# nzfeng/signed-heat-3d

Hardware: AMD Instinct MI355X
Metric: grid-nodes/sec end-to-end SHM (conv+PCG) (higher is better)
Workload: dtype f64 (Step 1: f64 / packed-f32 tiers)

## Files before the change

signed-heat-3d_amd/csrc/shm_conv_tiered.hip.h:

```cpp
#pragma once
#include "shm_far_carry.h"
#include "shm_kernels.hip.h"

namespace shm {

typedef unsigned uint2v __attribute__((ext_vector_type(2)));
constexpr double kNearA1 = 3.384507729693224e-04;
__device__ __forceinline__ double yukawa_near(double x, double c1, double c2, double m1, const uint2v* __restrict__ tab) {
    const double y0 = __builtin_amdgcn_rsq(x);
    const double t = x * y0;
    const double e2 = fma(-t, y0, 1.0);
    const double cc = fma(e2, c2, c1);
    const double tm = fma(-t, cc, m1);
    const double kf = tm - m1;
    const unsigned ki = (unsigned)__double_as_longlong(tm);
    const double f = fma(-t, cc, -kf);
    const double q = y0 * cc;
    double p = 5.727446245172041e-08;
    p = fma(p, f, kNearA1);
    p = fma(p, f, 1.0);
    uint2v tv = tab[ki & 2047u];
    tv.y += ki << 9;
    return __builtin_bit_cast(double, tv) * (p * q);
}

template <int B>
__device__ __forceinline__ void yukawa_near_batch(const double* __restrict__ x, double c1, double c2, double m1, const uint2v* __restrict__ tab, double* __restrict__ g) {
    double y0[B], t[B], cc[B], q[B], tm[B], f[B], p[B];
    unsigned ki[B];
    uint2v tv[B];
#pragma unroll
    for (int b = 0; b < B; b++) y0[b] = __builtin_amdgcn_rsq(x[b]);
#pragma unroll
    for (int b = 0; b < B; b++) t[b] = x[b] * y0[b];
#pragma unroll
// ... 111 lines not shown
#define SHM_TIER_WAVES_PER_EU 2
#endif
template <int NPT, typename TY, bool CHECK>
__global__ __launch_bounds__(kBlock) __attribute__((amdgpu_waves_per_eu(SHM_TIER_WAVES_PER_EU, SHM_TIER_WAVES_PER_EU))) void conv_tiered_kernel(
    ConvParams P, const double* __restrict__ src , const float* __restrict__ clusters,
    const double* __restrict__ exp_tab_g , TY* __restrict__ Y0, TY* __restrict__ Y1, TY* __restrict__ Y2,
    unsigned long long* __restrict__ counters, unsigned* __restrict__ next_unit ) {
    static_assert(NPT % 2 == 0, "the far tier handles a lane's nodes in packed pairs");
    constexpr int kWaves = kBlock / kWave;
    constexpr int kFarUnroll = SHM_TIER_FAR_UNROLL;
    static_assert(kFarUnroll == kFarGroup, "the carry's bookkeeping (shm_far_carry.h) counts in groups of the far loop's unroll");
    constexpr int kFarList = kTierCluster + kFarGroup;
    static_assert((kTierCluster + kFarGroup - 1 + kFarGroup - 1) / kFarGroup * kFarGroup <= kFarList, "carry + cluster + padding fit the far lists");
    __shared__ double stage64[kWaves][kTierCluster * 6];
    __shared__ __attribute__((aligned(16))) float farA[kWaves][kFarList * 4];
    __shared__ __attribute__((aligned(16))) float farB[kWaves][kFarList * NPT];
    __shared__ __attribute__((aligned(16))) float farC[kWaves][kFarList * 2];
#if SHM_TIER_LDS_FETCH
    __shared__ double2 raw[kWaves][3][kTierCluster];
#endif
    __shared__ uint2v exp_tab[2048];
    __shared__ float4 star_stash[kWaves];
    const int wave = __builtin_amdgcn_readfirstlane((int)(threadIdx.x >> 6)), lane = (int)(threadIdx.x & 63);
    double* const tile = stage64[wave];
    float* const tA = farA[wave];
    float* const tB = farB[wave];
    float* const tC = farC[wave];
    for (int a = threadIdx.x; a < 2048; a += kBlock) {
        uint2v tv = __builtin_bit_cast(uint2v, exp_tab_g[a]);
        tv.y -= (unsigned)a << 9;
        exp_tab[a] = tv;
    }
    __syncthreads();
    const int n = P.n;
    const size_t plane = (size_t)n * n;
    const float lam_l2 = (float)(P.lambda * 1.4426950408889634);
    const float g_l2 = P.tier_log * 1.4426950408889634f;
    const bool drop_on = P.drop_eps_soft > 0.f;
    const float cellq = (float)(P.cell * (P.lambda * 1.4426950408889634));
    const float lws = uniform_f32((float)log2(P.wscale));
    constexpr double kHalfZ = 0.5 * (NPT - 1);
    constexpr double kHalfX = 0.5 * (kTierTX - 1), kHalfY = 0.5 * (kTierTY - 1);
    const float rt_w = (float)(sqrt(kHalfX * kHalfX + kHalfY * kHalfY + kHalfZ * kHalfZ) * P.cell) * 1.000001f;
    const float hx = uniform_f32((float)(kHalfX * P.cell) * 1.000001f), hy = uniform_f32((float)(kHalfY * P.cell) * 1.000001f),
                hz = uniform_f32((float)(kHalfZ * P.cell) * 1.000001f);
    const double c1 = -P.cexp, c2 = -0.5 * P.cexp;
    unsigned long long cnt_near = 0, cnt_far = 0, cnt_redo = 0;
    int decided = -1;
    const unsigned n_units = (unsigned)P.n_tiles;
    const unsigned per_q = (n_units + 7u) / 8u;
    const unsigned my_q = blockIdx.x & 7u;
    unsigned q_off = 0;
    for (;;) {
        unsigned unit = 0xffffffffu;
        while (q_off < 8u) {
            const unsigned q = (my_q + q_off) & 7u;
            const unsigned lo = q * per_q, hi = min(n_units, lo + per_q);
            unsigned t = 0;
            if (lane == 0) t = atomicAdd(next_unit + q, 1u);
            t = (unsigned)__builtin_amdgcn_readfirstlane((int)t);
            if (lo + t < hi) {
                unit = lo + t;
                break;
            }
            q_off++;
        }
        if (unit == 0xffffffffu) break;
        const int tzq = (int)(unit / (unsigned)(P.tiles_x * P.tiles_y)), trem = (int)unit - tzq * (P.tiles_x * P.tiles_y);
        const int tz = P.layer_order ? P.layer_order[tzq] : tzq;
        bool use_diff = false;
// ... 79 lines not shown

        const int k0 = __builtin_amdgcn_readfirstlane((int)floor((double)d0_w * P.cexp * (1.0 / 2048.0)));
        const double m1 = 6755399441055744.0 - 2048.0 * (double)k0;
        auto far_scale = [&]() {
            float d = d0_w;
            asm volatile("" : "+v"(d));
            return exp2_tab(fma((double)d, P.cexp, -2048.0 * (double)k0), exp_tab) * (P.lambda * 1.4426950408889634) / P.wscale;
        };
        float2v fl[NPT / 2];
#pragma unroll
        for (int e = 0; e < NPT / 2; e++) fl[e] = float2v{0.f, 0.f};
        const float range_c = uniform_f32(2.f * rt_w * lam_l2 - 113.f - coff);
        float star_ux = 0.f, star_uy = 0.f, star_uz = 0.f, star_dc = 0.f, star_inv_d = 0.f;
        if constexpr (CHECK) {
            use_diff = use_diff && coff + 2.f * rt_w * lam_l2 <= 72.f;
        }
        if (use_diff || drop_on) {
            const float inv = dmin > 0.f ? 1.f / dmin : 0.f;
            star_ux = uniform_f32(nx * inv);
            star_uy = uniform_f32(ny * inv);
            star_uz = uniform_f32(nz * inv);
            star_dc = uniform_f32(dmin * 1.000001f);
            const float bx = fmaxf(fabsf(nx) - hx, 0.f), by = fmaxf(fabsf(ny) - hy, 0.f), bz = fmaxf(fabsf(nz) - hz, 0.f);
            const float db = sqrtf(bx * bx + by * by + bz * bz);
            star_inv_d = uniform_f32(dmin > 0.f && db > 0.f ? 1.f / db : __builtin_huge_valf());
        }
        float R_soft = 0.f, R_hard = 0.f;
        if constexpr (CHECK) {
            if (drop_on && lane == 0) star_stash[wave] = float4{(cx - nx) * lam_l2, (cy - ny) * lam_l2, (cz - nz) * lam_l2, wnear};
        }
        const float span_c = uniform_f32(2.f * rt_w * lam_l2 - coff - 960.f);
        int far_pending = 0;
        int carry = 0;
#pragma unroll 1
        for (int pass = 0; pass < 2; pass++) {
#if SHM_TIER_LDS_FETCH
        auto fetch_cluster = [&](int c) {
            const char* g = reinterpret_cast<const char*>(src) + (size_t)c * (kTierCluster * 48);
            const unsigned lo = (unsigned)lane * 48u;
            __builtin_amdgcn_global_load_lds(g + lo, &raw[wave][0][0], 16, 0, 0);
            __builtin_amdgcn_global_load_lds(g + 16 + lo, &raw[wave][1][0], 16, 0, 0);
            __builtin_amdgcn_global_load_lds(g + 32 + lo, &raw[wave][2][0], 16, 0, 0);
        };
#else
        double nq[6];
        auto fetch_cluster = [&](int c) {
            const double* qn = src + ((size_t)c * kTierCluster + lane) * 6;
#pragma unroll
            for (int a = 0; a < 6; a++) nq[a] = qn[a];
        };
#endif
        int cur_batch = -1;
        unsigned long long kept_mask = 0ull, cdrop_mask = 0ull;
        auto load_batch = [&](int b) {
            cur_batch = b;
            const int ci = b * kWave + lane;
            const bool in = ci < P.n_clusters;
            const unsigned long long validm = __ballot(in);
            cdrop_mask = 0ull;
            if (drop_on) {
                const float2* rec = reinterpret_cast<const float2*>(clusters + (size_t)min(ci, P.n_clusters - 1) * kConvClusterRec);
                const float2 r0 = rec[0], r1 = rec[1], r2 = rec[2];
                const float gdx = cx - r0.x, gdy = cy - r0.y, gdz = cz - r1.x;
                const float gap = sqrtf(gdx * gdx + gdy * gdy + gdz * gdz) * 0.999999f - rt_w - r1.y - r_hi_w;
                const float lrel = lws - lnear_w - gap * lam_l2;
                const float lbmax = fmaf(r2.x, 1.4426950408889634f, lrel) + 2e-5f;
                const bool cand = in && gap > 0.f && lbmax <= P.drop_ltau;
                const unsigned long long candm = __ballot(cand);
                if (candm != 0ull) {
                    float bc = cand ? __builtin_amdgcn_exp2f(fmaf(r2.y, 1.4426950408889634f, lrel)) * (r_hi_w * __builtin_amdgcn_rcpf(r_hi_w + gap)) * 1.0001f : 0.f;
                    bc += __int_as_float(__builtin_amdgcn_ds_swizzle(__float_as_int(bc), 0x1f | (1 << 10)));
                    bc += __int_as_float(__builtin_amdgcn_ds_swizzle(__float_as_int(bc), 0x1f | (2 << 10)));
                    bc += __int_as_float(__builtin_amdgcn_ds_swizzle(__float_as_int(bc), 0x1f | (4 << 10)));
                    bc += __int_as_float(__builtin_amdgcn_ds_swizzle(__float_as_int(bc), 0x1f | (8 << 10)));
                    bc += __int_as_float(__builtin_amdgcn_ds_swizzle(__float_as_int(bc), 0x1f | (16 << 10)));
                    const float sum = __int_as_float(__builtin_amdgcn_readlane(__float_as_int(bc), 0)) + __int_as_float(__builtin_amdgcn_readlane(__float_as_int(bc), 32));
                    const float r_new = uniform_f32(R_soft + sum);
                    if (__builtin_amdgcn_readfirstlane((int)(r_new <= P.drop_eps_soft))) {
                        R_soft = r_new;
                        cdrop_mask = candm;
                    } else {
                        cdrop_mask = __ballot(cand && lbmax <= P.drop_ltau_hard);
                        R_hard = uniform_f32(R_hard + (float)(__builtin_popcountll(cdrop_mask) * kTierCluster) * P.drop_tau_hard);
                    }
                }
            }
            kept_mask = pass == 1 ? validm : validm & ~cdrop_mask;
        };
        auto next_kept = [&](int from, bool& cdrop) {
            cdrop = false;
#pragma unroll 1
            while (from < P.n_clusters) {
                const int b = from >> 6;
                if (b != cur_batch) load_batch(b);
                const unsigned long long m = kept_mask & (~0ull << (from & 63));
                if (m != 0ull) {
                    const int bit = (int)__builtin_ctzll(m);
                    cdrop = ((cdrop_mask >> bit) & 1ull) != 0ull;
                    return (b << 6) + bit;
                }
                from = (b + 1) << 6;
            }
            return P.n_clusters;
        };
        R_soft = 0.f;
        R_hard = 0.f;
        bool cdrop_cur = false, cdrop_next = false;
        int c = next_kept(0, cdrop_cur);
        if (c < P.n_clusters) fetch_cluster(c);
#pragma unroll 1
        while (c < P.n_clusters) {
            const int c_next = next_kept(c + 1, cdrop_next);
            const int c_fetch = c_next;
            double q[6];
#if SHM_TIER_LDS_FETCH
            {
                __builtin_amdgcn_s_waitcnt(0x0f70);
                const double2 r0 = raw[wave][0][lane], r1 = raw[wave][1][lane], r2 = raw[wave][2][lane];
                q[0] = r0.x; q[1] = r0.y; q[2] = r1.x; q[3] = r1.y; q[4] = r2.x; q[5] = r2.y;
                __builtin_amdgcn_s_waitcnt(0xc07f);
// ... 4 lines not shown
#endif
            if (c_fetch < P.n_clusters) fetch_cluster(c_fetch);
            unsigned long long nearmask, farmask;
            {
                float q32[6];
#pragma unroll
                for (int a = 0; a < 6; a++) q32[a] = a < 3 ? (float)q[a] : (float)(q[a] * P.wscale);
                const float dx = fmaxf(fabsf(cx - q32[0]) - hx, 0.f), dy = fmaxf(fabsf(cy - q32[1]) - hy, 0.f), dz = fmaxf(fabsf(cz - q32[2]) - hz, 0.f);
                const float dist = sqrtf(dx * dx + dy * dy + dz * dz);
                const float w2 = q32[3] * q32[3] + q32[4] * q32[4] + q32[5] * q32[5];
                const float lw = 0.5f * __log2f(w2);
                const float rel = lw + 1e-5f - lnear_w;
                const float lhs = (dist * 0.999999f - r_hi_w) * lam_l2;
                const bool valid = q[3] != 0. || q[4] != 0. || q[5] != 0.;
                const bool in_range = fmaf(dist, lam_l2, range_c) <= lw;
                float lhs_far = lhs, lhs_drop = lhs;
                {
                    bool want_diff = use_diff;
                    if (!want_diff && drop_on && !cdrop_cur) {
                        const float lb_box = rel - lhs;
                        want_diff = __ballot(valid && lb_box > P.drop_ltau && lb_box <= P.drop_ltau + 2.02f * rt_w * lam_l2) != 0ull;
                    }
                    if (want_diff) {
                        const float ex = cx - q32[0], ey = cy - q32[1], ez = cz - q32[2];
                        const float dc2 = ex * ex + ey * ey + ez * ez, rdc = __builtin_amdgcn_rsqf(dc2), dc = dc2 * rdc;
                        const float dot = (ex * star_ux + ey * star_uy + ez * star_uz) * rdc;
                        const float du = sqrtf(fmaxf(0.f, 2.f - 2.f * dot));
                        const float lip = du + rt_w * (__builtin_amdgcn_rcpf(dist) + star_inv_d);
                        const float lhs2 = (dc * 0.999999f - star_dc - rt_w * lip * 1.00001f) * lam_l2;
                        lhs_drop = fmaxf(lhs, lhs2);
                        if (use_diff) lhs_far = lhs_drop;
                    }
                }
                const bool far = lhs_far > g_l2 + rel && in_range && (!CHECK || dist >= r_hi_w);
                bool drop = valid && cdrop_cur;
                if (drop_on && !cdrop_cur) {
                    const float lb = rel - lhs_drop + 2e-5f;
                    const bool cand = valid && lb <= P.drop_ltau;
                    if (__ballot(cand) != 0ull) {
                        float bs = cand ? __builtin_amdgcn_exp2f(lb) * (r_hi_w * __builtin_amdgcn_rcpf(dist)) * 1.0001f : 0.f;
                        bs += __int_as_float(__builtin_amdgcn_ds_swizzle(__float_as_int(bs), 0x1f | (1 << 10)));
                        bs += __int_as_float(__builtin_amdgcn_ds_swizzle(__float_as_int(bs), 0x1f | (2 << 10)));
                        bs += __int_as_float(__builtin_amdgcn_ds_swizzle(__float_as_int(bs), 0x1f | (4 << 10)));
                        bs += __int_as_float(__builtin_amdgcn_ds_swizzle(__float_as_int(bs), 0x1f | (8 << 10)));
                        bs += __int_as_float(__builtin_amdgcn_ds_swizzle(__float_as_int(bs), 0x1f | (16 << 10)));
                        const float sum = __int_as_float(__builtin_amdgcn_readlane(__float_as_int(bs), 0)) + __int_as_float(__builtin_amdgcn_readlane(__float_as_int(bs), 32));
                        const float r_new = uniform_f32(R_soft + sum);
                        if (__builtin_amdgcn_readfirstlane((int)(r_new <= P.drop_eps_soft))) {
                            R_soft = r_new;
                            drop = cand;
                        } else {
                            drop = cand && lb <= P.drop_ltau_hard && dist >= r_hi_w;
                            R_hard = uniform_f32(R_hard + (float)__builtin_popcountll(__ballot(drop)) * P.drop_tau_hard);
                        }
                    }
                }
                const bool span_ok = fmaf(dist, lam_l2, span_c) < 0.f;
                const bool to64 = valid && (pass == 0 ? (!drop && !far) : (drop ? span_ok : true));
                const bool to32 = valid && pass == 0 && far && !drop;
                nearmask = __ballot(to64);
                farmask = __ballot(to32);
                if (to64) {
                    const int rnk = mask_rank(nearmask);
#pragma unroll
                    for (int a = 0; a < 6; a++) tile[rnk * 6 + a] = a < 3 ? q[a] : q[a] * P.cexp_inv;
                } else if (to32) {
                    const int rnk = carry + mask_rank(farmask);
                    *reinterpret_cast<float4*>(&tA[rnk * 4]) = float4{q32[0] * lam_l2, q32[1] * lam_l2, q32[3], q32[4]};
                    const float dz0 = qz0 - q32[2] * lam_l2;
                    float dz2[NPT];
#pragma unroll
                    for (int e = 0; e < NPT; e++) {
                        const float dz = e * cellq + dz0;
                        dz2[e] = dz * dz;
                    }
                    if constexpr (NPT == 4) *reinterpret_cast<float4*>(&tB[rnk * 4]) = float4{dz2[0], dz2[1], dz2[2], dz2[3]};
                    else *reinterpret_cast<float2*>(&tB[rnk * 2]) = float2{dz2[0], dz2[1]};
                    *reinterpret_cast<float2*>(&tC[rnk * 2]) = float2{q32[5], fabsf(q32[3]) + fabsf(q32[4]) + fabsf(q32[5])};
                }
            }
            const int nnear = __builtin_popcountll(nearmask), nfar = __builtin_popcountll(farmask);
            const FarCarryStep fs = far_carry_step(carry, nfar, far_pending, CHECK ? P.tier_flush : 0, c_next >= P.n_clusters);
            if (lane < fs.pad) {
                const int at = carry + nfar + lane;
                *reinterpret_cast<float4*>(&tA[at * 4]) = float4{1.0e18f, 1.0e18f, 0.f, 0.f};
#pragma unroll
                for (int e = 0; e < NPT; e++) tB[at * NPT + e] = 1.0e36f;
                *reinterpret_cast<float2*>(&tC[at * 2]) = float2{0.f, 0.f};
            }
            cnt_near += (unsigned)nnear;
            cnt_far += (unsigned)nfar;
            if (pass) cnt_redo += (unsigned)nnear;
            auto near_source = [&](const double (&rec)[6]) {
                const double dx = px - rec[0], dy = py - rec[1];
                const double dxy2 = dx * dx + dy * dy;
                const double dz0 = pz0 - rec[2];
                double x[NPT], g[NPT];
#pragma unroll
                for (int e = 0; e < NPT; e++) {
                    const double dz = e == 2 ? fma(2.0, P.cell, dz0) : e ? dz0 + e * P.cell : dz0;
                    x[e] = fma(dz, dz, dxy2);
                }
                constexpr int kB = SHM_TIER_NEAR_BATCH < NPT ? SHM_TIER_NEAR_BATCH : NPT;
#pragma unroll
                for (int b0 = 0; b0 < NPT; b0 += kB) yukawa_near_batch<kB>(x + b0, c1, c2, m1, exp_tab, g + b0);
#pragma unroll
                for (int e = 0; e < NPT; e++) {
                    ax[e] = fma(rec[3], g[e], ax[e]);
                    ay[e] = fma(rec[4], g[e], ay[e]);
                    az[e] = fma(rec[5], g[e], az[e]);
                }
            };
            for (int i0 = 0; i0 < nnear; i0++) {
                double rec[6];
#pragma unroll
                for (int a = 0; a < 6; a++) rec[a] = tile[6 * i0 + a];
                near_source(rec);
            }
            for (int i0f = 0; i0f < fs.run; i0f += kFarUnroll) {
                constexpr int kP = kFarUnroll * (NPT / 2);
                float2v wxy[kFarUnroll], pcw[kFarUnroll], d2[kP], rinv[kP], g[kP];
                float dxy2[kFarUnroll];
#pragma unroll
                for (int u = 0; u < kFarUnroll; u++) {
                    const int s = i0f + u;
// ... 34 lines not shown
                if (fs.flush) {
                    const double e0f = far_scale();
#pragma unroll
                    for (int e = 0; e < NPT; e++) {
                        ax[e] = fma((double)fx[e / 2][e & 1], e0f, ax[e]);
                        ay[e] = fma((double)fy[e / 2][e & 1], e0f, ay[e]);
                        az[e] = fma((double)fz[e / 2][e & 1], e0f, az[e]);
                    }
#pragma unroll
                    for (int e = 0; e < NPT / 2; e++) fx[e] = fy[e] = fz[e] = float2v{0.f, 0.f};
                }
            }
            if (fs.carry > 0 && fs.run > 0) {
                if (lane < fs.carry) {
                    const int from = fs.run + lane;
                    const float4 ca = *reinterpret_cast<const float4*>(&tA[from * 4]);
                    const float2 cc2 = *reinterpret_cast<const float2*>(&tC[from * 2]);
                    if constexpr (NPT == 4) {
                        const float4 cb = *reinterpret_cast<const float4*>(&tB[from * 4]);
                        *reinterpret_cast<float4*>(&tB[lane * 4]) = cb;
                    } else {
                        const float2 cb = *reinterpret_cast<const float2*>(&tB[from * 2]);
                        *reinterpret_cast<float2*>(&tB[lane * 2]) = cb;
                    }
                    *reinterpret_cast<float4*>(&tA[lane * 4]) = ca;
                    *reinterpret_cast<float2*>(&tC[lane * 2]) = cc2;
                }
            }
            carry = fs.carry;
            c = c_next;
            cdrop_cur = cdrop_next;
        }
        if (!CHECK) break;
        if (pass == 0) {
            bool fail = false;
            const double e0 = far_scale();
            const float r_drop = R_soft + R_hard;
            const float4 st = star_stash[wave];
            float chk = P.drop_check, k0_here = (float)k0;
            asm volatile("" : "+v"(chk), "+v"(k0_here));
            const float rs = r_drop * chk * 1.01f * sqrtf(st.w) * __builtin_amdgcn_exp2f(-lws) * lam_l2;
            const float sdx = qx - st.x, sdy = qy - st.y, sdz0 = qz0 - st.z;
            const float ratio_f = uniform_f32((float)P.far_redo_ratio * (P.tier_u0 > 0.f ? fminf(1.f, P.tier_u0 / (coff + g_l2)) : 1.f));
            const float sxy2 = sdx * sdx + sdy * sdy;
#pragma unroll
            for (int e = 0; e < NPT; e++) {
                const double x0 = ax[e] + (double)fx[e / 2][e & 1] * e0, x1 = ay[e] + (double)fy[e / 2][e & 1] * e0, x2 = az[e] + (double)fz[e / 2][e & 1] * e0;
                const float dz = e * cellq + sdz0, d2 = fmaf(dz, dz, sxy2), rinv = __builtin_amdgcn_rsqf(d2);
                const float tstar = r_drop > 0.f ? rs * __builtin_amdgcn_exp2f(-d2 * rinv - k0_here) * rinv : 0.f;
                fail = fail || (live_xy && kk0 + e < P.kk_end && fma((double)fl[e / 2][e & 1], e0, (double)tstar) > (double)ratio_f * sqrt(x0 * x0 + x1 * x1 + x2 * x2));
            }
            if (__ballot(fail) == 0ull) break;
#pragma unroll
            for (int e = 0; e < NPT / 2; e++) fx[e] = fy[e] = fz[e] = float2v{0.f, 0.f};
#pragma unroll
            for (int e = 0; e < NPT; e++) ax[e] = ay[e] = az[e] = 0.;
        }
        }
        const double e0 = far_scale();
        int lane_here = lane;
        asm volatile("" : "+v"(lane_here));
        const int si = min(i0 + (lane_here % kTierTX), n - 1), sj = min(j0 + (lane_here / kTierTX), n - 1);
#pragma unroll
        for (int e = 0; e < NPT; e++) {
            if (!(live_xy && kk0 + e < P.kk_end)) continue;
            const int kback = sizeof(TY) == 8 ? k0 : 0;
            const double x0 = __builtin_amdgcn_ldexp(ax[e] + (double)fx[e / 2][e & 1] * e0, kback), x1 = __builtin_amdgcn_ldexp(ay[e] + (double)fy[e / 2][e & 1] * e0, kback),
                         x2 = __builtin_amdgcn_ldexp(az[e] + (double)fz[e / 2][e & 1] * e0, kback);
            const double nrm = sqrt(x0 * x0 + x1 * x1 + x2 * x2);
            const size_t vi = (size_t)(kk0 + e) * plane + (size_t)sj * n + si;
            Y0[vi] = (TY)(x0 / nrm);
            Y1[vi] = (TY)(x1 / nrm);
            Y2[vi] = (TY)(x2 / nrm);
        }
        if constexpr (CHECK) {
            if (rule_sel == 1 && lane == 0)
                sample_report(P.sample_ctr, (cnt_far - far_before) * (unsigned long long)(64 * NPT), (cnt_redo - redo_before) * (unsigned long long)(64 * NPT), P.sample_blocks);
        }
    }
    if (counters && lane == 0) {
        atomicAdd(&counters[0], cnt_near * (unsigned long long)(64 * NPT));
        atomicAdd(&counters[1], cnt_far * (unsigned long long)(64 * NPT));
        if (cnt_redo) atomicAdd(&counters[2], cnt_redo * (unsigned long long)(64 * NPT));
    }
}

}
// ... 1 lines not shown
```

signed-heat-3d_amd/csrc/shm_grid.hip:

```cpp
#include "shm_host.hip.h"
#include "shm_audit_sample.h"


struct shm_solver {
    std::unique_ptr<shm::SolverBase> impl;
    std::string err;
    shm_config cfg;
};

static thread_local std::string g_create_error;

template <typename F> static shm_status guard(shm_solver* s, F&& f) {
    if (!s) return SHM_ERR_INVALID;
    try {
        f();
        s->err.clear();
        return SHM_OK;
    } catch (const shm::Error& e) {
        s->err = e.what();
        return e.code;
    } catch (const std::bad_alloc&) {
        s->err = "host allocation failed";
        return SHM_ERR_NOMEM;
    } catch (const std::exception& e) {
        s->err = e.what();
        return SHM_ERR_INVALID;
    }
}

extern "C" {

int32_t shm_grid_abi_version(void) { return SHM_GRID_ABI_VERSION; }

void shm_plan_slab(int32_t n, int32_t nslabs, int32_t slab, int32_t* k0, int32_t* k1) {
    if (nslabs < 1 || n < 0 || slab < 0 || slab >= nslabs) {
        if (k0) *k0 = 0;
        if (k1) *k1 = 0;
        return;
    }
    const int32_t q = n / nslabs, r = n % nslabs;
    const int32_t b = slab * q + (slab < r ? slab : r);
    if (k0) *k0 = b;
    if (k1) *k1 = b + q + (slab < r ? 1 : 0);
}

shm_status shm_step1_plane_weights(const shm_sources* src, const shm_grid* grid, int32_t precision, double* weights) {
    if (!src || !grid || !weights || src->S <= 0 || !src->pos || !src->wnormal || grid->n < 1 || !(grid->cell > 0.) || !(src->lambda > 0.) ||
        (precision != SHM_F64 && precision != SHM_F32))
        return SHM_ERR_INVALID;
    const char* tl = shm::knob("SHM_CONV_TIER_LOG");
    try {
        shm::step1_plane_weights_host(src->S, src->pos, src->wnormal, src->lambda, grid->n, grid->bbox_min, grid->cell, precision, tl ? atof(tl) : 8.0, weights,
                                      precision == SHM_F32 && shm::knob("SHM_CONV32_CLASSIC") == nullptr);
    } catch (const std::bad_alloc&) {
        return SHM_ERR_NOMEM;
    } catch (...) {
        return SHM_ERR_INVALID;
    }
    return SHM_OK;
}

void shm_plan_slab_weighted(int32_t n, int32_t nslabs, int32_t slab, const double* weights, int32_t granule, int32_t* k0, int32_t* k1) {
    if (k0) *k0 = 0;
    if (k1) *k1 = 0;
    if (nslabs < 1 || n < nslabs || slab < 0 || slab >= nslabs) return;
    try {
        std::vector<int32_t> b;
        shm::plan_slabs_weighted(n, nslabs, weights, granule, b);
        if (k0) *k0 = b[(size_t)slab];
        if (k1) *k1 = b[(size_t)slab + 1];
    } catch (...) {
    }
}

shm_status shm_grid_create(const shm_config* cfg, shm_solver** out) {
    if (!cfg || !out) {
        g_create_error = "null argument";
        return SHM_ERR_INVALID;
    }
    *out = nullptr;
    try {
        shm_config c = *cfg;
        if (c.local_slabs <= 0) c.local_slabs = 1;
        if (c.world <= 0) c.world = 1;
        if (c.rank < 0 || c.rank >= c.world) throw shm::Error(SHM_ERR_INVALID, "rank out of range");
// ... 217 lines not shown
```

signed-heat-3d_amd/csrc/shm_host.hip.h:

```cpp
#pragma once
#include <hip/hip_runtime.h>
#include <rccl/rccl.h>

#include <dlfcn.h>

#include <algorithm>
#include <atomic>
#include <chrono>
#include <cmath>
#include <cstdarg>
#include <cstdio>
#include <cstring>
#include <limits>
#include <memory>
#include <mutex>
#include <stdexcept>
#include <string>
#include <thread>
#include <unordered_map>
#include <unordered_set>
#include <vector>

#include "../../include/shm_grid.h"
#include "shm_constraints.h"

namespace shm {

struct Error : std::runtime_error {
    shm_status code;
    Error(shm_status c, const std::string& m) : std::runtime_error(m), code(c) {}
};

static const char* knob(const char* name) {
    static const bool on = getenv("SHM_DEBUG_KNOBS") != nullptr && atoi(getenv("SHM_DEBUG_KNOBS")) != 0;
    return on ? getenv(name) : nullptr;
}

static std::string fmt(const char* f, ...) {
    char buf[1024];
    va_list ap;
    va_start(ap, f);
    vsnprintf(buf, sizeof buf, f, ap);
    va_end(ap);
    return buf;
}

#define HIPCHK(expr)                                                                                         \
    do {                                                                                                     \
        hipError_t e_ = (expr);                                                                              \
        if (e_ != hipSuccess)                                                                                \
            throw shm::Error(e_ == hipErrorOutOfMemory ? SHM_ERR_NOMEM : SHM_ERR_HIP,                        \
                             shm::fmt("%s failed: %s (%s:%d)", #expr, hipGetErrorString(e_), __FILE__, __LINE__)); \
    } while (0)

struct Rccl {
    typedef ncclComm_t comm_t;
    typedef ncclUniqueId unique_id;
// ... 486 lines not shown
```

signed-heat-3d_amd/csrc/shm_kernels.hip.h:

```cpp
#pragma once
#include <hip/hip_runtime.h>
#include <stdint.h>

#include <type_traits>

#include "shm_constraints.h"
#include "shm_mc_table.h"

namespace shm {

constexpr int kBlock = 256;
constexpr int kMaxPartials = 8192;

__device__ __forceinline__ double wave_sum(double v) {
#pragma unroll
    for (int off = 32; off > 0; off >>= 1) v += __shfl_down(v, off, kWave);
    return v;
}

__device__ __forceinline__ double block_sum(double v, double* lds ) {
    v = wave_sum(v);
    const int lane = threadIdx.x & 63, w = threadIdx.x >> 6;
    if (lane == 0) lds[w] = v;
    __syncthreads();
// ... 55 lines not shown
        return __builtin_amdgcn_ldexp(p, (int)kf);
    }
};
template <> struct YukawaMath<float> {
    static __device__ __forceinline__ void rsqrt_and_sqrt(float x, float& rinv, float& r) {
        const float y0 = __builtin_amdgcn_rsqf(x);
        r = x * y0;
        rinv = y0;
    }
    static __device__ __forceinline__ float exp_neg(float x) { return __expf(x); }
};
template <typename T> __device__ __forceinline__ T t_rcp(T x);
template <> __device__ __forceinline__ double t_rcp<double>(double x) { return __builtin_amdgcn_rcp(x); }
template <> __device__ __forceinline__ float t_rcp<float>(float x) { return __builtin_amdgcn_rcpf(x); }
template <typename T> __device__ __forceinline__ T t_sqrt(T x);
template <> __device__ __forceinline__ double t_sqrt<double>(double x) { return sqrt(x); }
template <> __device__ __forceinline__ float t_sqrt<float>(float x) { return sqrtf(x); }

struct ConvParams {
    int n;
    int kk_begin;
    int kk_end;
    int k0;
    int tiles_x, tiles_y;
    double bbox_min[3];
    double cell;
    double lambda;
    double cexp;
    double cexp_inv;
    int S;
    int n_clusters;
    float far_gap;
    float tier_log;
    float skip_base;
    float inv_lambda;
    int exact_offset;
    int n_tiles;
    double wscale;
    float far_redo_ratio;
    int far_rule;
    const unsigned char* unit_rule;
    unsigned long long* sample_ctr;
    int sample_blocks;
    const int* layer_order;
    float drop_eps_soft, drop_ltau, drop_ltau_hard, drop_tau_hard;
    float tier_u0;
    int tier_flush;
    float drop_check;
};

typedef float float2v __attribute__((ext_vector_type(2)));
constexpr int kConvTile = 8;
template <typename T> constexpr int conv_cluster() { return sizeof(T) == 8 ? 64 : 32; }
template <typename T> constexpr int conv_chunk() { return (sizeof(T) == 8 ? kSrcTile : 4 * kSrcTile) / conv_cluster<T>(); }
constexpr int kConvClusterRec = 6;

#ifndef SHM_CONV32_UNROLL
#define SHM_CONV32_UNROLL 2
#endif
template <int NPT> struct ConvSrcUnroll { static constexpr int value = NPT == 8 ? SHM_CONV32_UNROLL : 2; };
template <typename T, int NPT>
__global__ __launch_bounds__(kBlock) void conv_normalize_kernel(ConvParams P, const T* __restrict__ src ,
                                                                const float* __restrict__ src32, const float* __restrict__ clusters,
                                                                const double* __restrict__ exp_tab_g ,
                                                                T* __restrict__ Y0, T* __restrict__ Y1, T* __restrict__ Y2,
                                                                unsigned long long* __restrict__ counters ,
// ... 1779 lines not shown
```

signed-heat-3d_amd/csrc/shm_solver.hip.h:

```cpp
#pragma once
#include "shm_host.hip.h"
#include "shm_kernels.hip.h"
#include "shm_conv_tiered.hip.h"
#include "shm_cg_fused.hip.h"
#include "shm_twolevel.hip.h"
#include "shm_schur.hip.h"
#include "shm_dct.hip.h"
#include "shm_dct_gemm.hip.h"
#include "shm_green_fft.hip.h"
#include "shm_sample.hip.h"
#include "shm_audit.hip.h"
#include "shm_iso_indexed.hip.h"
#include "shm_iso_components.hip.h"
#include "shm_raycast.hip.h"
#include "shm_redistance.hip.h"
#include "shm_redistance_exact.hip.h"
#include "shm_closest.hip.h"
#include "shm_plan.h"

namespace shm {

template <typename T> constexpr int vec_width() { return sizeof(T) == 8 ? 2 : 4; }

template <typename T>
// ... 16 lines not shown
    int sample_blocks = 0;
    long long layer_order_key = -1;
    DevArray<double> div_partials;
    int div_sum_blocks = 0;
    DevArray<T> touched_save;
    DevArray<T> W1, W2;
    DevArray<T> S1, S2, S4;
    DevArray<int> act_x, act_y;
    DevArray<unsigned> act_z;
    DevArray<int> act_planes;
    int n_act_planes = 0;
    int n_act_x = 0, n_act_y = 0;
    int n_touched = 0, n_shift = 0;
    GridParams gp{};
};

template <typename T>
struct Solver final : SolverBase {
    shm_config cfg;
    hipStream_t stream = nullptr;
    hipStream_t stream2 = nullptr;
    hipStream_t stream3 = nullptr;
    std::unique_ptr<Event> e_sch_in, e_sch_done, e_gs_done;
    hipStream_t stream_h = nullptr;
    int n = 0, alloc_n = -1;
    size_t N = 0;
    double cell = 0., lambda = 0.;
    double bbox_min[3] = {0, 0, 0};
    double conv_ctr[3] = {0, 0, 0};
    double conv_wscale = 1.;
    int64_t S = 0;
    std::vector<double> h_pos, h_wn, h_area;
    double area_sum = 0., conv_far_gap = 0., conv_skip_base = 3.0e38, last_host_setup_ms = 0., last_setup_wall_ms = 0.;
    double conv_tier_log = 0., conv_tier_skip_base = 3.0e38;
    double conv_drop_K = 64., conv_drop_eps64 = 2e-9, conv_drop_eps32 = 6.0e-8;
    double conv_w_span = 0.;
    DevArray<double> d_src_t;
    DevArray<float> d_clusters_t;
    int n_clusters_t = 0;
    bool conv_tiered = false;
    bool conv_tier_exact = false;
    bool conv_tiered32 = false;
    bool conv_reference = false;
    int step1_selected = SHM_STEP1_AUTO;
    int last_step1_arith = SHM_STEP1_AUTO;
    double last_step1_budget = 0.;
    bool fold_pq = false;
    int fold_pq_np = 0;
    double step1_budget = 0.;
    DevArray<unsigned long long> d_pair_counters;
    DevArray<unsigned> d_unit_counters;
    static constexpr int kMaxConvLaunches = 256;
    int conv_launch_index = 0;
    int conv_launches_last = 0;
    int n_clusters = 0;
    int conv_grid_cap = 1 << 30;
    bool o_fast_hint = false;
    int num_cus = 256;
    DevArray<T> d_src;
    DevArray<float> d_src32;
    DevArray<float> d_clusters;
    DevArray<double> d_exptab;
    std::vector<Slab<T>> slabs;
    int total_slabs = 1, first_slab = 0;
    std::vector<int32_t> slab_bounds;
    bool slabs_equal = true;
// ... 203 lines not shown
                    for (int a = 0; a < 3; a++) cc[a] += (double)packed[6 * ((size_t)c * kConvCluster + e) + a];
                for (int a = 0; a < 3; a++) cc[a] /= kConvCluster;
                double rad = 0.;
                for (int e = 0; e < kConvCluster; e++) {
                    double d2 = 0.;
                    for (int a = 0; a < 3; a++) {
                        const double d = (double)packed[6 * ((size_t)c * kConvCluster + e) + a] - cc[a];
                        d2 += d * d;
                    }
                    rad = std::max(rad, std::sqrt(d2));
                }
                for (int a = 0; a < 3; a++) cl[kConvClusterRec * (size_t)c + a] = (float)cc[a];
                cl[kConvClusterRec * (size_t)c + 3] = (float)(rad * 1.00001 + 1e-30);
                double wmax2 = 0., wsum = 0.;
                for (int e = 0; e < kConvCluster; e++) {
                    double w2 = 0.;
                    for (int a = 0; a < 3; a++) {
                        const double w = (double)packed[6 * ((size_t)c * kConvCluster + e) + 3 + a];
                        w2 += w * w;
                    }
                    wmax2 = std::max(wmax2, w2);
                    wsum += std::sqrt(w2);
                }
                cl[kConvClusterRec * (size_t)c + 4] = wmax2 > 0. ? (float)(0.5 * std::log(wmax2) + 1e-5) : -1.0e30f;
                cl[kConvClusterRec * (size_t)c + 5] = wsum > 0. ? (float)(std::log(wsum) + 1e-5) : -1.0e30f;
            }
            {
                const double far_log = 25.0;
                conv_far_gap = (far_log + std::log(std::max(1.0, amax / std::max(amin, 1e-300)))) / lambda;
                const double eps = sizeof(T) == 8 ? 1.1e-16 : 6.0e-8;
                const char* sk = knob("SHM_CONV_NO_SKIP");
                conv_skip_base = sk ? 3.0e38 : std::log((double)S / eps);
                const char* tl = knob("SHM_CONV_TIER_LOG");
                conv_tier_log = tl ? atof(tl) : 8.0;
                conv_tier_skip_base = sk ? 3.0e38 : std::log((double)S / 2e-9);
                conv_drop_eps64 = sk ? 0. : 2e-9;
                conv_drop_eps32 = sk ? 0. : 6.0e-8;
                conv_drop_K = drop_rule_K(S, h_wn.data(), lambda);
                select_step1_arith(SHM_STEP1_AUTO);
            }
            d_src.upload(packed, stream);
            d_src32.upload(packed32, stream);
            {
                const int per = conv_chunk<T>();
                const int nchunks = (n_clusters + per - 1) / per;
                for (int g = 0; g < nchunks; g++) {
                    const int a = g * per, b = std::min(n_clusters, a + per);
                    double cc[3] = {0, 0, 0};
                    for (int c = a; c < b; c++)
                        for (int t = 0; t < 3; t++) cc[t] += cl[kConvClusterRec * (size_t)c + t];
                    for (int t = 0; t < 3; t++) cc[t] /= (b - a);
                    double rad = 0., lnw = -1.0e30;
                    for (int c = a; c < b; c++) {
                        double d2 = 0.;
                        for (int t = 0; t < 3; t++) {
                            const double d = (double)cl[kConvClusterRec * (size_t)c + t] - cc[t];
                            d2 += d * d;
                        }
                        rad = std::max(rad, std::sqrt(d2) + (double)cl[kConvClusterRec * (size_t)c + 3]);
                        lnw = std::max(lnw, (double)cl[kConvClusterRec * (size_t)c + 4]);
                    }
                    for (int t = 0; t < 3; t++) cl.push_back((float)cc[t]);
                    cl.push_back((float)(rad * 1.00001 + 1e-30));
                    cl.push_back((float)lnw);
                    cl.push_back(0.f);
                }
            }
// ... 252 lines not shown
        }
        return true;
    }
    void launch_conv() {
        const bool slab_log = knob("SHM_CONV_SLAB_LOG") != nullptr;
        Event slab_ev[2];
        unsigned long long slab_pairs_seen[2] = {0, 0};
        for (Slab<T>& sl : slabs) {
            if (slab_log) {
                HIPCHK(hipStreamSynchronize(stream));
                slab_ev[0].record(stream);
            }
            ConvParams P;
            P.layer_order = nullptr;
            P.unit_rule = nullptr;
            P.sample_ctr = nullptr;
            P.sample_blocks = 0;
            P.far_rule = conv_tiered && !conv_tier_exact && sizeof(T) == 8 ? far_rule_now() : 0;
            P.n = n;
            P.kk_begin = 1;
            P.kk_end = sl.nzl + 1;
            P.k0 = sl.k0;
            for (int a = 0; a < 3; a++) P.bbox_min[a] = bbox_min[a] - conv_ctr[a];
            P.cell = cell;
            P.lambda = lambda;
            P.cexp = -lambda * 2954.639443740597;
            P.cexp_inv = 1.0 / std::fabs(P.cexp);
            P.S = n_clusters * conv_cluster<T>();
            P.n_clusters = n_clusters;
            P.far_gap = conv_reference ? 3.0e38f : (float)conv_far_gap;
            const double budget = step1_budget > 0. ? step1_budget : kTierBudget;
            const double g_shift = std::log(budget / kTierBudget);
            P.tier_log = conv_tier_exact ? 3.0e38f : conv_tiered32 ? -1.0e30f : (float)std::max(2.0, conv_tier_log - g_shift);
            P.wscale = conv_wscale;
            {
                const double ratio = budget / kTierEpsFar;
                P.far_redo_ratio = ratio > 0. ? (float)ratio : 3.0e38f;
            }
            P.skip_base = conv_tier_exact || conv_reference ? 3.0e38f : (float)std::min(conv_tiered ? conv_tier_skip_base - g_shift : conv_skip_base, 3.0e38);
            {
                const double eps = conv_tier_exact ? 0. : sizeof(T) == 8 ? conv_drop_eps64 * (budget / kTierBudget) : conv_drop_eps32;
                const double eps_soft = 0.875 * eps, tau = eps_soft / conv_drop_K, tau_hard = 0.125 * eps / (double)std::max<int64_t>(1, S);
                P.drop_eps_soft = (float)eps_soft;
                P.drop_ltau = eps > 0. ? (float)std::log2(tau) : -3.0e38f;
                P.drop_ltau_hard = eps > 0. ? (float)std::log2(tau_hard) : -3.0e38f;
                P.drop_tau_hard = (float)(tau_hard * 1.0001);
                P.drop_check = P.far_redo_ratio < 1.0e30f ? (float)((double)P.far_redo_ratio / budget) : (float)(1.0 / kTierEpsFar);
                P.tier_u0 = (float)kTierU0;
                P.tier_flush = kTierFlush;
            }
            P.inv_lambda = (float)(1.0 / lambda);
            P.tiles_x = (n + kConvTile - 1) / kConvTile;
            P.tiles_y = P.tiles_x;
            const int planes = P.kk_end - P.kk_begin;
            const bool npt4 = (long long)P.tiles_x * P.tiles_y * ((planes + 15) / 16) >= conv_grid_cap;
            const bool npt4_env = knob("SHM_CONV_NPT4") != nullptr;
            const bool npt8 = sizeof(T) == 4 && !npt4_env && npt4 && (long long)P.tiles_x * P.tiles_y * ((planes + 31) / 32) >= conv_grid_cap;
            const int tile_z = npt8 ? 32 : npt4 ? 16 : 8;
            const double half_z = 0.5 * ((npt8 ? 16 : tile_z) - 1);
            const double tile_diam = 2.0 * std::sqrt(2 * 3.5 * 3.5 + half_z * half_z) * cell;
            P.exact_offset = (lambda * tile_diam > 30.0) ? 1 : 0;
            const int tiles_z = (planes + tile_z - 1) / tile_z;
            P.n_tiles = P.tiles_x * P.tiles_y * tiles_z;
            unsigned grid = (unsigned)std::min(P.n_tiles, conv_grid_cap);
            {
                int occ = 0;
// ... 2986 lines not shown
```

Baseline: 688.9 million.

## Add intermediate ring pass with wider f32 tier threshold before full-f64 redo

Adds a middle pass to the tiered convolution: when the first tiered pass fails its error check, it retries with the far threshold widened by a ring margin, so only nearer clusters move to f64, rather than recomputing everything in f64. A 'hopeless' test skips the ring pass when the dropped-mass bound alone would still fail. The aim is to cut the cost of full-f64 redos on tiles that barely fail. The risk is a third pass on tiles that fail both tiered passes, plus a stray s_nop sequence and extra register pressure.

```diff
diff --git a/signed-heat-3d_amd/csrc/shm_conv_tiered.hip.h b/signed-heat-3d_amd/csrc/shm_conv_tiered.hip.h
--- a/signed-heat-3d_amd/csrc/shm_conv_tiered.hip.h
+++ b/signed-heat-3d_amd/csrc/shm_conv_tiered.hip.h
@@ -1,6 +1,7 @@
 #pragma once
 #include "shm_far_carry.h"
 #include "shm_kernels.hip.h"
+#include "shm_tier_passes.h"
 
 namespace shm {
 
@@ -178,10 +179,12 @@
         exp_tab[a] = tv;
     }
     __syncthreads();
+    asm volatile("s_nop 0\n s_nop 0\n s_nop 0\n s_nop 0\n s_nop 0\n s_nop 0");
     const int n = P.n;
     const size_t plane = (size_t)n * n;
     const float lam_l2 = (float)(P.lambda * 1.4426950408889634);
     const float g_l2 = P.tier_log * 1.4426950408889634f;
+    const float ring_l2 = CHECK ? P.tier_ring * 1.4426950408889634f : 0.f;
     const bool drop_on = P.drop_eps_soft > 0.f;
     const float cellq = (float)(P.cell * (P.lambda * 1.4426950408889634));
     const float lws = uniform_f32((float)log2(P.wscale));
@@ -327,8 +330,11 @@
         const float span_c = uniform_f32(2.f * rt_w * lam_l2 - coff - 960.f);
         int far_pending = 0;
         int carry = 0;
+        bool drop_fails = false;
 #pragma unroll 1
-        for (int pass = 0; pass < 2; pass++) {
+        for (int pass = kTierPassFirst; pass <= kTierPassAllF64; pass++) {
+        if (!tier_pass_runs(pass, ring_l2, drop_fails)) continue;
+        const TierPass tp = tier_pass(pass, CHECK, g_l2, ring_l2);
 #if SHM_TIER_LDS_FETCH
         auto fetch_cluster = [&](int c) {
             const char* g = reinterpret_cast<const char*>(src) + (size_t)c * (kTierCluster * 48);
@@ -380,7 +386,7 @@
                     }
                 }
             }
-            kept_mask = pass == 1 ? validm : validm & ~cdrop_mask;
+            kept_mask = tp.tiered ? validm & ~cdrop_mask : validm;
         };
         auto next_kept = [&](int from, bool& cdrop) {
             cdrop = false;
@@ -451,7 +457,7 @@
                         if (use_diff) lhs_far = lhs_drop;
                     }
                 }
-                const bool far = lhs_far > g_l2 + rel && in_range && (!CHECK || dist >= r_hi_w);
+                const bool far = lhs_far > tp.g_l2 + rel && in_range && (!CHECK || dist >= r_hi_w);
                 bool drop = valid && cdrop_cur;
                 if (drop_on && !cdrop_cur) {
                     const float lb = rel - lhs_drop + 2e-5f;
@@ -475,8 +481,8 @@
                     }
                 }
                 const bool span_ok = fmaf(dist, lam_l2, span_c) < 0.f;
-                const bool to64 = valid && (pass == 0 ? (!drop && !far) : (drop ? span_ok : true));
-                const bool to32 = valid && pass == 0 && far && !drop;
+                const bool to64 = valid && (tp.tiered ? (!drop && !far) : (drop ? span_ok : true));
+                const bool to32 = valid && tp.tiered && far && !drop;
                 nearmask = __ballot(to64);
                 farmask = __ballot(to32);
                 if (to64) {
@@ -509,7 +515,7 @@
             }
             cnt_near += (unsigned)nnear;
             cnt_far += (unsigned)nfar;
-            if (pass) cnt_redo += (unsigned)nnear;
+            if (tp.redo) cnt_redo += (unsigned)nnear;
             auto near_source = [&](const double (&rec)[6]) {
                 const double dx = px - rec[0], dy = py - rec[1];
                 const double dxy2 = dx * dx + dy * dy;
@@ -610,7 +616,7 @@
             cdrop_cur = cdrop_next;
         }
         if (!CHECK) break;
-        if (pass == 0) {
+        if (tp.test) {
             bool fail = false;
             const double e0 = far_scale();
             const float r_drop = R_soft + R_hard;
@@ -619,18 +625,24 @@
             asm volatile("" : "+v"(chk), "+v"(k0_here));
             const float rs = r_drop * chk * 1.01f * sqrtf(st.w) * __builtin_amdgcn_exp2f(-lws) * lam_l2;
             const float sdx = qx - st.x, sdy = qy - st.y, sdz0 = qz0 - st.z;
-            const float ratio_f = uniform_f32((float)P.far_redo_ratio * (P.tier_u0 > 0.f ? fminf(1.f, P.tier_u0 / (coff + g_l2)) : 1.f));
+            const float ratio_f = uniform_f32((float)P.far_redo_ratio * (P.tier_u0 > 0.f ? fminf(1.f, P.tier_u0 / (coff + tp.g_l2)) : 1.f));
             const float sxy2 = sdx * sdx + sdy * sdy;
+            const float ratio_ring = uniform_f32((float)P.far_redo_ratio * (P.tier_u0 > 0.f ? fminf(1.f, P.tier_u0 / (coff + tp.g_l2 + ring_l2)) : 1.f));
+            bool hopeless = false;
 #pragma unroll
             for (int e = 0; e < NPT; e++) {
                 const double x0 = ax[e] + (double)fx[e / 2][e & 1] * e0, x1 = ay[e] + (double)fy[e / 2][e & 1] * e0, x2 = az[e] + (double)fz[e / 2][e & 1] * e0;
                 const float dz = e * cellq + sdz0, d2 = fmaf(dz, dz, sxy2), rinv = __builtin_amdgcn_rsqf(d2);
                 const float tstar = r_drop > 0.f ? rs * __builtin_amdgcn_exp2f(-d2 * rinv - k0_here) * rinv : 0.f;
-                fail = fail || (live_xy && kk0 + e < P.kk_end && fma((double)fl[e / 2][e & 1], e0, (double)tstar) > (double)ratio_f * sqrt(x0 * x0 + x1 * x1 + x2 * x2));
+                const double nrm = sqrt(x0 * x0 + x1 * x1 + x2 * x2);
+                fail = fail || (live_xy && kk0 + e < P.kk_end && fma((double)fl[e / 2][e & 1], e0, (double)tstar) > (double)ratio_f * nrm);
+                hopeless = hopeless || (live_xy && kk0 + e < P.kk_end && (double)tstar > (double)ratio_ring * nrm);
             }
             if (__ballot(fail) == 0ull) break;
-#pragma unroll
-            for (int e = 0; e < NPT / 2; e++) fx[e] = fy[e] = fz[e] = float2v{0.f, 0.f};
+            drop_fails = __ballot(hopeless) != 0ull;
+#pragma unroll
+            for (int e = 0; e < NPT / 2; e++) fx[e] = fy[e] = fz[e] = fl[e] = float2v{0.f, 0.f};
+            far_pending = 0;
 #pragma unroll
             for (int e = 0; e < NPT; e++) ax[e] = ay[e] = az[e] = 0.;
         }
diff --git a/signed-heat-3d_amd/csrc/shm_grid.hip b/signed-heat-3d_amd/csrc/shm_grid.hip
--- a/signed-heat-3d_amd/csrc/shm_grid.hip
+++ b/signed-heat-3d_amd/csrc/shm_grid.hip
@@ -50,7 +50,7 @@
         return SHM_ERR_INVALID;
     const char* tl = shm::knob("SHM_CONV_TIER_LOG");
     try {
-        shm::step1_plane_weights_host(src->S, src->pos, src->wnormal, src->lambda, grid->n, grid->bbox_min, grid->cell, precision, tl ? atof(tl) : 8.0, weights,
+        shm::step1_plane_weights_host(src->S, src->pos, src->wnormal, src->lambda, grid->n, grid->bbox_min, grid->cell, precision, tl ? atof(tl) : shm::kTierLogDefault, weights,
                                       precision == SHM_F32 && shm::knob("SHM_CONV32_CLASSIC") == nullptr);
     } catch (const std::bad_alloc&) {
         return SHM_ERR_NOMEM;
diff --git a/signed-heat-3d_amd/csrc/shm_host.hip.h b/signed-heat-3d_amd/csrc/shm_host.hip.h
--- a/signed-heat-3d_amd/csrc/shm_host.hip.h
+++ b/signed-heat-3d_amd/csrc/shm_host.hip.h
@@ -23,6 +23,7 @@
 
 #include "../../include/shm_grid.h"
 #include "shm_constraints.h"
+#include "shm_tier_passes.h"
 
 namespace shm {
 
diff --git a/signed-heat-3d_amd/csrc/shm_kernels.hip.h b/signed-heat-3d_amd/csrc/shm_kernels.hip.h
--- a/signed-heat-3d_amd/csrc/shm_kernels.hip.h
+++ b/signed-heat-3d_amd/csrc/shm_kernels.hip.h
@@ -111,6 +111,7 @@
     int n_clusters;
     float far_gap;
     float tier_log;
+    float tier_ring;
     float skip_base;
     float inv_lambda;
     int exact_offset;
diff --git a/signed-heat-3d_amd/csrc/shm_solver.hip.h b/signed-heat-3d_amd/csrc/shm_solver.hip.h
--- a/signed-heat-3d_amd/csrc/shm_solver.hip.h
+++ b/signed-heat-3d_amd/csrc/shm_solver.hip.h
@@ -72,6 +72,7 @@
     int64_t S = 0;
     std::vector<double> h_pos, h_wn, h_area;
     double area_sum = 0., conv_far_gap = 0., conv_skip_base = 3.0e38, last_host_setup_ms = 0., last_setup_wall_ms = 0.;
+    double conv_tier_ring = 0.;
     double conv_tier_log = 0., conv_tier_skip_base = 3.0e38;
     double conv_drop_K = 64., conv_drop_eps64 = 2e-9, conv_drop_eps32 = 6.0e-8;
     double conv_w_span = 0.;
@@ -341,7 +342,9 @@
                 const char* sk = knob("SHM_CONV_NO_SKIP");
                 conv_skip_base = sk ? 3.0e38 : std::log((double)S / eps);
                 const char* tl = knob("SHM_CONV_TIER_LOG");
-                conv_tier_log = tl ? atof(tl) : 8.0;
+                conv_tier_log = tl ? atof(tl) : kTierLogDefault;
+                const char* tr = knob("SHM_CONV_TIER_RING");
+                conv_tier_ring = std::max(0.0, tr ? atof(tr) : kTierRingDefault);
                 conv_tier_skip_base = sk ? 3.0e38 : std::log((double)S / 2e-9);
                 conv_drop_eps64 = sk ? 0. : 2e-9;
                 conv_drop_eps32 = sk ? 0. : 6.0e-8;
@@ -660,6 +663,7 @@
             const double budget = step1_budget > 0. ? step1_budget : kTierBudget;
             const double g_shift = std::log(budget / kTierBudget);
             P.tier_log = conv_tier_exact ? 3.0e38f : conv_tiered32 ? -1.0e30f : (float)std::max(2.0, conv_tier_log - g_shift);
+            P.tier_ring = conv_tier_exact || conv_tiered32 ? 0.f : (float)conv_tier_ring;
             P.wscale = conv_wscale;
             {
                 const double ratio = budget / kTierEpsFar;
diff --git a/signed-heat-3d_amd/csrc/shm_tier_passes.h b/signed-heat-3d_amd/csrc/shm_tier_passes.h
--- /dev/null
+++ b/signed-heat-3d_amd/csrc/shm_tier_passes.h
@@ -0,0 +1,34 @@
+#pragma once
+
+#ifdef __HIPCC__
+#define SHM_TIER_PASSES_HD __host__ __device__ __forceinline__
+#else
+#define SHM_TIER_PASSES_HD inline
+#endif
+
+namespace shm {
+
+constexpr double kTierLogDefault = 8.0;
+constexpr double kTierRingDefault = 2.0;
+
+constexpr int kTierPassFirst = 0, kTierPassRing = 1, kTierPassAllF64 = 2;
+
+struct TierPass {
+    bool tiered;
+    float g_l2;
+    bool test;
+    bool redo;
+};
+
+SHM_TIER_PASSES_HD TierPass tier_pass(int pass, bool check, float g_l2, float ring_l2) {
+    TierPass t;
+    t.tiered = !check || pass != kTierPassAllF64;
+    t.g_l2 = pass == kTierPassRing ? g_l2 + ring_l2 : g_l2;
+    t.test = check && t.tiered;
+    t.redo = pass != kTierPassFirst;
+    return t;
+}
+
+SHM_TIER_PASSES_HD bool tier_pass_runs(int pass, float ring_l2, bool drop_fails) { return pass != kTierPassRing || (ring_l2 > 0.f && !drop_fails); }
+
+}
```

New measurement: 698.3 million (median of 6 runs). 1.01x the previous value.
